# michaelklachko/NoisyNet

Measured on AMD Instinct MI355X. Metric: images/sec (whole node) + top-1, NoisyNet 4-bit CIFAR-10 I_max=1nA, 1/2/4/8 GPU, higher is better.
Workload: dtype bf16; 1 GPU; model=noisynet-4layer-cifar, global_batch=32768, image_size=32, augment=True, hip_graph=False, q_a=4, q_w=0, current_nA=1, act_max=5, optim=adamw, parallelism=dp1

## Files before the change

### __graft_entry__.py

```python
#!/usr/bin/env python3

import glob
import os
import shutil
import sys

REPO = os.path.dirname(os.path.abspath(__file__))
sys.path.insert(0, REPO)


def build():
    os.environ.setdefault("PYTORCH_ROCM_ARCH", "gfx950")

    sources = sorted(glob.glob(os.path.join(REPO, "csrc", "*.hip")))
    sources += sorted(glob.glob(os.path.join(REPO, "csrc", "*.cpp")))
    build_dir = os.path.join(REPO, "build")
    os.makedirs(build_dir, exist_ok=True)
    _build_manual(build_dir, sources)

    so_src = os.path.join(build_dir, "noisynet_hip.so")
    so_dst = os.path.join(REPO, "noisynet_amd", "ops", "noisynet_hip.so")
    if os.path.exists(so_src):
        shutil.copy2(so_src, so_dst)

    import noisynet_amd

    from noisynet_amd.ops import _ext
    mod = _ext.ext()
    for sym in ("conv_fwd_fused", "conv_wgrad_patch", "set_seed_buffer",
                "softmax_xent_bwd_t", "bn_stats_finalize", "dwconv_wgrad",
                "crop_resize_mirror_normalize", "conv_fused_route",
                "linear_fused_route", "xbar_fwd_conv", "xbar_fwd_linear",
                "xbar_diff_fwd_conv", "xbar_diff_fwd_linear",
                "xbar_serial_fwd_conv", "xbar_serial_fwd_linear"):
        if not hasattr(mod, sym):
            raise RuntimeError("build(): %s missing from %s -- stale build"
                               % (sym, so_dst))
    print("build(): extension built at", so_dst)


def _build_manual(build_dir, sources):
    import subprocess

    import torch
    from torch.utils import cpp_extension as ce

    torch_lib = os.path.join(os.path.dirname(torch.__file__), "lib")
    includes = ce.include_paths(device_type="cuda")
    inc_flags = ["-I" + p for p in includes]
# ... 104 lines not shown
```

### csrc/bindings.cpp

```cpp

#include <torch/extension.h>

torch::Tensor fake_quant_fwd(torch::Tensor x, int64_t num_bits, double min_value,
                             double max_value, double stochastic, int64_t seed);
torch::Tensor ste_mask(torch::Tensor grad, torch::Tensor x, double min_value,
                       double max_value);
torch::Tensor mult_uniform_noise(torch::Tensor x, double a, int64_t seed);
torch::Tensor relu_clip_fwd(torch::Tensor x, bool relu, double act_max);
torch::Tensor relu_clip_bwd(torch::Tensor g, torch::Tensor y, bool relu,
                            double act_max);
std::vector<torch::Tensor> dropout_fwd(torch::Tensor x, double p, int64_t seed);
void set_seed_buffer(torch::Tensor t);
void clear_seed_buffer();

void sgd_step(torch::Tensor p, torch::Tensor g, torch::Tensor buf, double lr,
              double momentum, double wd, bool nesterov, double cmin,
              double cmax);
void adamw_step(torch::Tensor p, torch::Tensor g, torch::Tensor m,
                torch::Tensor v, int64_t step, double lr, double beta1,
                double beta2, double eps, double wd, double cmin, double cmax);

std::vector<torch::Tensor> softmax_xent_fwd(torch::Tensor logits,
                                            torch::Tensor target);
torch::Tensor softmax_xent_bwd(torch::Tensor softmax, torch::Tensor target,
// ... 12 lines not shown
std::vector<torch::Tensor> bn_act_bwd(torch::Tensor g, torch::Tensor x,
                                      torch::Tensor y, torch::Tensor mean,
                                      torch::Tensor invstd, torch::Tensor gamma,
                                      bool training, bool relu,
                                      double act_max);
std::vector<torch::Tensor> bn_act_bwd_reduce(torch::Tensor g, torch::Tensor x,
                                             torch::Tensor y, torch::Tensor mean,
                                             torch::Tensor invstd, bool relu,
                                             double act_max);
torch::Tensor bn_act_bwd_apply(torch::Tensor g, torch::Tensor x,
                               torch::Tensor y, torch::Tensor mean,
                               torch::Tensor invstd, torch::Tensor gamma,
                               torch::Tensor sum_g, torch::Tensor sum_gx,
                               double count, bool training, bool relu,
                               double act_max);

std::vector<torch::Tensor> maxpool2x2_fwd(torch::Tensor x);
torch::Tensor maxpool2x2_bwd(torch::Tensor g, torch::Tensor code, int64_t H,
                             int64_t W);
std::vector<torch::Tensor> maxpool_fwd(torch::Tensor x, int64_t k,
                                       int64_t stride, int64_t pad);
torch::Tensor maxpool_bwd(torch::Tensor g, torch::Tensor code, int64_t H,
                          int64_t W, int64_t k, int64_t stride, int64_t pad);
torch::Tensor avgpool_fwd(torch::Tensor x, int64_t k, int64_t stride,
                          int64_t pad);
torch::Tensor avgpool_bwd(torch::Tensor g, int64_t H, int64_t W, int64_t k,
                          int64_t stride, int64_t pad);

torch::Tensor dwconv_fwd(torch::Tensor x, torch::Tensor w, torch::Tensor bias,
                         int64_t stride, int64_t pad);
// ... 13 lines not shown
                                           torch::Tensor meta,
                                           int64_t out_size,
                                           std::vector<double> mean,
                                           std::vector<double> std,
                                           int64_t out_dtype);

torch::Tensor kth_percentile(torch::Tensor x, double pctl);

torch::Tensor conv_fwd(torch::Tensor x, torch::Tensor w, int64_t stride,
                       int64_t pad);
std::vector<torch::Tensor> conv_fwd_fused(torch::Tensor x, torch::Tensor wq,
                                          torch::Tensor wraw, torch::Tensor bias,
                                          int64_t stride, int64_t pad,
                                          int64_t sigma_mode,
                                          torch::Tensor factor,
                                          int64_t seed, bool telem);
torch::Tensor conv_dgrad(torch::Tensor gy, torch::Tensor w, int64_t stride,
                         int64_t pad, int64_t H, int64_t W);
torch::Tensor conv_wgrad(torch::Tensor gy, torch::Tensor x, int64_t stride,
                         int64_t pad, int64_t R, int64_t S);
torch::Tensor im2col_materialize(torch::Tensor x, int64_t K, int64_t stride,
                                 int64_t pad, int64_t R, int64_t S);
torch::Tensor conv_wgrad_from_col(torch::Tensor gy, torch::Tensor col,
                                  int64_t C, int64_t R, int64_t S);
torch::Tensor conv_wgrad_im2col(torch::Tensor gy, torch::Tensor x,
                                int64_t stride, int64_t pad, int64_t R,
                                int64_t S);
torch::Tensor conv_wgrad_patch(torch::Tensor gy, torch::Tensor x,
                               int64_t stride, int64_t pad, int64_t R,
                               int64_t S,
                               c10::optional<torch::Tensor> x_padded);
// ... 80 lines not shown
  m.def("relu_clip_bwd", &relu_clip_bwd);
  m.def("dropout_fwd", &dropout_fwd);
  m.def("set_seed_buffer", &set_seed_buffer);
  m.def("clear_seed_buffer", &clear_seed_buffer);
  m.def("sgd_step", &sgd_step);
  m.def("adamw_step", &adamw_step);
  m.def("softmax_xent_fwd", &softmax_xent_fwd);
  m.def("softmax_xent_bwd", &softmax_xent_bwd);
  m.def("softmax_xent_bwd_t", &softmax_xent_bwd_t);
  m.def("bn_stats", &bn_stats);
  m.def("bn_stats_finalize", &bn_stats_finalize);
  m.def("bn_act_fwd", &bn_act_fwd);
  m.def("bn_act_bwd", &bn_act_bwd);
  m.def("bn_act_bwd_reduce", &bn_act_bwd_reduce);
  m.def("bn_act_bwd_apply", &bn_act_bwd_apply);
  m.def("maxpool2x2_fwd", &maxpool2x2_fwd);
  m.def("maxpool2x2_bwd", &maxpool2x2_bwd);
  m.def("dwconv_fwd", &dwconv_fwd);
  m.def("dwconv_dgrad", &dwconv_dgrad);
  m.def("dwconv_wgrad", &dwconv_wgrad);
  m.def("act_fwd", &act_fwd);
  m.def("act_bwd", &act_bwd);
  m.def("se_scale_fwd", &se_scale_fwd);
  m.def("se_scale_bwd", &se_scale_bwd);
  m.def("maxpool_fwd", &maxpool_fwd);
  m.def("maxpool_bwd", &maxpool_bwd);
  m.def("avgpool_fwd", &avgpool_fwd);
  m.def("avgpool_bwd", &avgpool_bwd);
  m.def("kth_percentile", &kth_percentile);
  m.def("crop_resize_mirror_normalize", &crop_resize_mirror_normalize);
  m.def("conv_fwd", &conv_fwd);
  m.def("conv_fwd_fused", &conv_fwd_fused);
  m.def("conv_dgrad", &conv_dgrad);
  m.def("conv_wgrad", &conv_wgrad);
  m.def("conv_wgrad_im2col", &conv_wgrad_im2col);
  m.def("conv_wgrad_patch", &conv_wgrad_patch, py::arg("gy"), py::arg("x"),
        py::arg("stride"), py::arg("pad"), py::arg("R"), py::arg("S"),
        py::arg("x_padded") = py::none());
  m.def("conv_wgrad_route", &conv_wgrad_route);
  m.def("conv_wgrad_from_col", &conv_wgrad_from_col);
  m.def("conv_pool_eligible", &conv_pool_eligible);
  m.def("conv_fused_route", &conv_fused_route);
  m.def("linear_fused_route", &linear_fused_route);
  m.def("conv_patch_tile", &conv_patch_tile);
  m.def("conv_pool_fwd_fused", &conv_pool_fwd_fused);
  m.def("conv_pool_wgrad", &conv_pool_wgrad);
  m.def("im2col_materialize", &im2col_materialize);
// ... 14 lines not shown
```

### csrc/bn_act.hip

```cpp

#include <torch/extension.h>
#include <ATen/ATen.h>
#include <c10/hip/HIPStream.h>
#include "common.h"

namespace {

constexpr int kBlock = 256;

template <typename T>
struct alignas(16) BnPack8 { T v[8]; };

template <typename T>
__global__ void bn_stats_kernel(const T* __restrict__ x,
                                float* __restrict__ partial_sum,
                                float* __restrict__ partial_sumsq,
                                int64_t rows, int C) {
  __shared__ float ls[kBlock], lsq[kBlock];
  int cbase = blockIdx.x * 64;
  int cw = C - cbase;
  if (cw > 64) cw = 64;
  int c_l = (cw == 64) ? (threadIdx.x & 63) : (threadIdx.x % cw);
  int rgrp = (cw == 64) ? (threadIdx.x >> 6) : (threadIdx.x / cw);
  int ngrp = kBlock / cw;
// ... 129 lines not shown
    outa[c] = sa;
    outb[c] = sb;
  }
}

template <typename T>
__global__ void bn_act_fwd_kernel(const T* __restrict__ x, T* __restrict__ y,
                                  const float* __restrict__ mean,
                                  const float* __restrict__ invstd,
                                  const float* __restrict__ gamma,
                                  const float* __restrict__ beta, int64_t n,
                                  int C, int do_relu, float act_max) {
  for (int64_t i = (int64_t)blockIdx.x * blockDim.x + threadIdx.x; i < n;
       i += (int64_t)gridDim.x * blockDim.x) {
    int c = (int)(i % C);
    float v = (to_f32(x[i]) - mean[c]) * invstd[c] * gamma[c] + beta[c];
    if (do_relu) v = fmaxf(v, 0.0f);
    if (act_max > 0.0f) v = fminf(v, act_max);
    y[i] = from_f32<T>(v);
  }
}

template <typename T>
__global__ void bn_act_fwd_vec_kernel(const T* __restrict__ x,
                                      T* __restrict__ y,
                                      const float* __restrict__ mean,
                                      const float* __restrict__ invstd,
                                      const float* __restrict__ gamma,
                                      const float* __restrict__ beta,
                                      int64_t n_vec, int Cv, int do_relu,
                                      float act_max) {
  using V = BnPack8<T>;
  for (int64_t i = (int64_t)blockIdx.x * blockDim.x + threadIdx.x; i < n_vec;
       i += (int64_t)gridDim.x * blockDim.x) {
    int c0 = (int)(i % Cv) * 8;
    V xv = ((const V*)x)[i];
    V o;
#pragma unroll
    for (int u = 0; u < 8; ++u) {
      int c = c0 + u;
      float v = (to_f32(xv.v[u]) - mean[c]) * invstd[c] * gamma[c] + beta[c];
      if (do_relu) v = fmaxf(v, 0.0f);
      if (act_max > 0.0f) v = fminf(v, act_max);
      o.v[u] = from_f32<T>(v);
    }
    ((V*)y)[i] = o;
  }
}

template <typename scalar_t> struct DevT { using type = scalar_t; };
template <> struct DevT<at::BFloat16> { using type = __hip_bfloat16; };
template <> struct DevT<at::Half> { using type = _Float16; };

__global__ void bn_finalize_kernel(const float* __restrict__ partial_sum,
                                   const float* __restrict__ partial_sumsq,
                                   float* __restrict__ mean,
                                   float* __restrict__ invstd,
                                   float* __restrict__ running_mean,
                                   float* __restrict__ running_var, int gy,
// ... 651 lines not shown
```

### csrc/common.h

```cpp
#pragma once

#include <hip/hip_runtime.h>
#include <hip/hip_bf16.h>
#include <hip/hip_fp16.h>
#include <cmath>
#include <cstdint>

#define WAVE 64
#define DEV_INLINE __device__ __forceinline__

template <typename T> DEV_INLINE float to_f32(T v);
template <> DEV_INLINE float to_f32<float>(float v) { return v; }
template <> DEV_INLINE float to_f32<__hip_bfloat16>(__hip_bfloat16 v) {
  return __bfloat162float(v);
}
template <> DEV_INLINE float to_f32<_Float16>(_Float16 v) { return (float)v; }

template <typename T> DEV_INLINE T from_f32(float v);
template <> DEV_INLINE float from_f32<float>(float v) { return v; }
template <> DEV_INLINE __hip_bfloat16 from_f32<__hip_bfloat16>(float v) {
  return __float2bfloat16(v);
}
template <> DEV_INLINE _Float16 from_f32<_Float16>(float v) {
  return (_Float16)v;
}

template <typename scalar_t>
inline float stored_act_max(double act_max) {
  return static_cast<float>(
      static_cast<scalar_t>(static_cast<float>(act_max)));
}

struct Philox4 {
  uint32_t x, y, z, w;
};

DEV_INLINE uint32_t mulhilo(uint32_t a, uint32_t b, uint32_t* hip) {
  uint64_t p = (uint64_t)a * (uint64_t)b;
  *hip = (uint32_t)(p >> 32);
  return (uint32_t)p;
}

DEV_INLINE Philox4 philox4x32(uint64_t seed, uint64_t counter) {
  uint32_t c0 = (uint32_t)counter, c1 = (uint32_t)(counter >> 32);
  uint32_t c2 = 0u, c3 = 0u;
// ... 106 lines not shown
```

### csrc/conv_mfma.hip

```cpp

#include <torch/extension.h>
#include <ATen/ATen.h>
#include <c10/hip/HIPStream.h>
#include <cstdlib>
#include <cstring>
#include <string>
#include "common.h"

namespace {

constexpr int kBlock = 256;
constexpr int BM = 64;
constexpr int BN = 64;
constexpr int BK = 32;

using bf16 = __hip_bfloat16;
using bf16x8 = __attribute__((ext_vector_type(8))) __bf16;
using f16x8 = __attribute__((ext_vector_type(8))) _Float16;
using f32x4 = __attribute__((ext_vector_type(4))) float;
using f32x8 = __attribute__((ext_vector_type(8))) float;


template <typename T> struct Mma;

// ... 2394 lines not shown
  } else {
    TORCH_CHECK(false, "conv_fwd_patch: layer-fitted tiles are 16-bit only");
  }
}

torch::Tensor pad_cols8(const torch::Tensor& in, int64_t K8);

bool conv_pad_share_enabled() {
  const char* e = getenv("NOISYNET_CONV_PAD_SHARE");
  return e == nullptr || std::string(e) != "0";
}

std::vector<torch::Tensor> conv_fwd_fused_patch_impl(
    torch::Tensor x, torch::Tensor wq, torch::Tensor wraw, torch::Tensor bias,
    int64_t stride, int64_t pad, int64_t sigma_mode, torch::Tensor factor,
    int64_t seed, bool telem, bool want_y) {
  check_sigma_mode(sigma_mode, want_y, "conv_fwd_fused (patch route)");
  check_cl(x, "conv_fwd_patch x");
  auto g = make_geom((int)x.size(0), (int)x.size(2), (int)x.size(3),
                     (int)x.size(1), (int)wraw.size(0), (int)wraw.size(2),
                     (int)wraw.size(3), (int)stride, (int)pad);
  PatchGeom p;
  p.C_pad = (g.C + 7) & ~7;
  p.Wp = g.W + 2 * g.pad;
  p.Kr = g.S * p.C_pad;
  p.Krs = (p.Kr + 31) & ~31;
  p.MI = g.OH * g.OW;
  auto out = torch::empty({g.N, g.K, g.OH, g.OW},
                          x.options().memory_format(at::MemoryFormat::ChannelsLast));
  bool has_bias = bias.numel() > 0;
  torch::Tensor bias_f;
  if (has_bias) bias_f = bias.to(torch::kFloat32).contiguous();
  auto tele = telem
      ? [&] {
          auto t = torch::zeros({3}, x.options().dtype(torch::kFloat32));
          t[2] = -std::numeric_limits<float>::infinity();
          return t;
        }()
      : torch::empty({0}, x.options().dtype(torch::kFloat32));
  auto factor_f = factor.to(torch::kFloat32).reshape({1}).contiguous();
  const PatchTileChoice tile = patch_tile(g, (int)x.element_size(),
                                          (int)sigma_mode, telem, want_y);
  torch::Tensor x_pad = torch::empty({0}, x.options());
  if (want_y && sigma_mode > 0 && x.element_size() == 2 && (g.C & 7) != 0 &&
      conv_pad_share_enabled()) {
    x_pad = pad_cols8(x.permute({0, 2, 3, 1})
                          .reshape({(int64_t)g.N * g.H * g.W, (int64_t)g.C})
                          .contiguous(), p.C_pad);
    x = x_pad;
    g.C = p.C_pad;
  }
  int k_pad = tile.kind == PatchTile::Generic ? (g.K + BN - 1) / BN * BN
                                              : tile.nrows;
  auto wq_pad = want_y ? pad_weight_full(wq, p.C_pad, k_pad, p.Krs)
                       : torch::Tensor();
  auto wraw_pad = (sigma_mode > 0)
                      ? pad_weight_full(wraw, p.C_pad, k_pad, p.Krs)
                      : torch::Tensor();
  size_t lds = 0;
  dim3 grid((g.K + BN - 1) / BN, g.N);
// ... 84 lines not shown
  } else {
    r = sigma_noise_linear_impl(col, wraw_flat, sigma_mode, factor, seed,
                                telem);
  }
  auto out = r[0].view({g.N, g.OH, g.OW, g.K}).permute({0, 3, 1, 2});
  return {out, r[1], col};
}

}

std::vector<torch::Tensor> conv_fwd_fused(torch::Tensor x, torch::Tensor wq,
                                          torch::Tensor wraw, torch::Tensor bias,
                                          int64_t stride, int64_t pad,
                                          int64_t sigma_mode,
                                          torch::Tensor factor,
                                          int64_t seed, bool telem) {
  auto g = make_geom((int)x.size(0), (int)x.size(2), (int)x.size(3),
                     (int)x.size(1), (int)wraw.size(0), (int)wraw.size(2),
                     (int)wraw.size(3), (int)stride, (int)pad);
  auto empty = torch::empty({0}, x.options());
  switch (conv_route(g, (int)x.element_size())) {
    case ConvRoute::Patch: {
      auto r = conv_fwd_fused_patch_impl(x, wq, wraw, bias, stride, pad,
                                         sigma_mode, factor, seed, telem,
                                         true);
      return r;
    }
    case ConvRoute::ColSmallK:
    case ConvRoute::ColGemm:
      return conv_fwd_fused_col_impl(x, wq, wraw, bias, stride, pad,
                                     sigma_mode, factor, seed, telem,
                                     true);
    case ConvRoute::Stream:
      break;
  }
  auto r = conv_fwd_fused_impl(x, wq, wraw, bias, stride, pad, sigma_mode,
                               factor, seed, telem, true);
  return {r[0], r[1], empty};
}

// ... 350 lines not shown
}

std::string conv_wgrad_route(int64_t C, int64_t H, int64_t W, int64_t K,
                             int64_t R, int64_t S, int64_t stride,
                             int64_t pad, int64_t elem_size) {
  if (ww_forced_legacy()) return "legacy";
  return ww_plan(1, C, H, W, K, R, S, stride, pad, elem_size, nullptr)
             ? "window" : "legacy";
}

torch::Tensor conv_wgrad_patch(torch::Tensor gy, torch::Tensor x,
                               int64_t stride, int64_t pad, int64_t R,
                               int64_t S,
                               c10::optional<torch::Tensor> x_padded) {
  check_cl(gy, "conv_wgrad_patch gy");
  check_cl(x, "conv_wgrad_patch x");
  TORCH_CHECK(x.element_size() == 2, "conv_wgrad_patch: 16-bit only");
  int64_t N = x.size(0), C = x.size(1), H = x.size(2), W = x.size(3);
  int64_t K = gy.size(1), OH = gy.size(2), OW = gy.size(3);
  int64_t M = N * OH * OW;
  int64_t Cp = (C + 7) & ~7;
  int64_t CRSp = R * S * Cp;

  auto x2 = x.permute({0, 2, 3, 1}).reshape({N * H * W, C});
  torch::Tensor xp;
  if (x_padded.has_value() && x_padded->numel() > 0) {
    TORCH_CHECK(x_padded->dim() == 2 && x_padded->size(0) == N * H * W &&
                    x_padded->size(1) == Cp && x_padded->is_contiguous() &&
                    x_padded->scalar_type() == x.scalar_type() &&
                    x_padded->device() == x.device(),
                "conv_wgrad_patch: x_padded must be [N*H*W, round8(C)]");
    xp = *x_padded;
  } else {
    xp = (Cp == C) ? x2.contiguous() : pad_cols8(x2.contiguous(), Cp);
  }
  auto gy2 = gy.permute({0, 2, 3, 1}).reshape({M, K});
  int64_t Kp = (K + 7) & ~7;
  torch::Tensor gyp = (Kp == K) ? gy2.contiguous()
                                : pad_cols8(gy2.contiguous(), Kp);

  int ctiles = (int)((CRSp + 127) / 128);
  int ktiles = (int)((Kp + 127) / 128);
  int64_t mtotal = (M + WG_BK - 1) / WG_BK;
  int64_t target_z = std::max<int64_t>(1, 2048 / std::max(1, ctiles * ktiles));
  int chunks = (int)((mtotal + target_z - 1) / target_z);
  int mslices = (int)((mtotal + chunks - 1) / chunks);
  dim3 grid(ctiles, ktiles, mslices);
  size_t lds = (size_t)256 * WG_LSTR;
// ... 1209 lines not shown
```

### noisynet_amd/models/noisynet.py

```python

import torch
from torch import nn

from .. import ops
from ..hardware_model import NoisyConv2d, NoisyLinear, add_noise_calculate_power
from ..quant import QuantMeasure


class Net(nn.Module):
    def __init__(self, args=None):
        super().__init__()
        self.args = args
        self.create_dir = True

        if args.train_act_max:
            self.act_max1 = nn.Parameter(torch.Tensor([0]), requires_grad=True)
            self.act_max2 = nn.Parameter(torch.Tensor([0]), requires_grad=True)
            self.act_max3 = nn.Parameter(torch.Tensor([0]), requires_grad=True)
        if args.train_w_max:
            self.w_max1 = nn.Parameter(torch.Tensor([0]), requires_grad=True)
            self.w_min1 = nn.Parameter(torch.Tensor([0]), requires_grad=True)

        self.pool = nn.MaxPool2d(2, 2)
        self.relu = nn.ReLU()
# ... 110 lines not shown
                                         -(-q_a // 4)))
        flags = self._introspective_flags()
        if flags:
            raise ValueError(
                '--xbar_rows %d cannot be combined with --%s: that flag runs '
                'the introspective forward, which models one unbounded '
                'crossbar per layer' % (self.xbar_rows, flags[0]))

    def _conv1_pool_fused(self, x, i):
        a = self.args
        return (a.current1 > 0 and i >= 20 and not x.requires_grad
                and a.L3 == 0 and a.L4 == 0
                and getattr(a, 'L3_new', 0) == 0
                and ops.conv_pool_eligible(x, self.conv1.weight))

    def _noisy_layer_fused(self, x, layer, current, merged_dac, i, layer_num,
                           is_conv, pool=False):
        a = self.args
        w_raw = layer.weight
        wq, bias = layer.effective_weight()
        want_telemetry = i < 20
        with torch.no_grad():
            if merged_dac:
                w_max = w_raw.detach().abs().max()
                factor = 0.1 * w_max / current
                sigma_mode = 'abs'
                power_denom = (x.detach().max() * w_max if want_telemetry
                               else w_max)
            else:
                input_max = x.detach().max()
                factor = 0.1 * input_max / current
                sigma_mode = 'abs2'
                power_denom = input_max
        telem = ops.NoiseTelemetry() if want_telemetry else None
        if is_conv:
            conv = ops.fused_noisy_conv2d_pool if pool \
                else ops.fused_noisy_conv2d
            out = conv(
                x, wq, w_raw.detach(), bias, 1, 0, sigma_mode, factor,
                current=current, power_denom=power_denom,
                want_telemetry=want_telemetry, telemetry_out=telem)
        else:
            out = ops.fused_noisy_linear(
                x, wq, w_raw.detach(), bias, sigma_mode, factor,
                current=current, power_denom=power_denom,
                want_telemetry=want_telemetry, telemetry_out=telem)
        if want_telemetry and telem.power is not None:
            self.power[layer_num].append(float(telem.power))
            self.nsr[layer_num].append(float(telem.nsr))
            self.input_sparsity[layer_num].append(float(telem.input_sparsity))
        return out

    def _xbar_serial_args(self, layer_num):
        if self.xbar_dac_bits <= 0:
            return {}
        k = layer_num + 1
# ... 83 lines not shown
                                 args.merged_dac, i, 0, True)
            self.conv1_ = x
            x = ops.maxpool2x2(x)
        elif self._conv1_pool_fused(x, i):
            x = self._noisy_layer_fused(x, self.conv1, args.current1,
                                        args.merged_dac, i, 0, True, pool=True)
            self.conv1_ = None
        else:
            if args.current1 > 0:
                x = self._noisy_layer_fused(x, self.conv1, args.current1,
                                            args.merged_dac, i, 0, True)
            else:
                x = self.conv1(x)
            self.conv1_ = x
            x = ops.maxpool2x2(x)
        if args.batchnorm:
            x = self._bn_act(x, self.bn1, args.act_max1)
        else:
            x = ops.relu_clip(x, args.act_max1)
        if args.dropout_conv > 0:
            x = ops.dropout(x, args.dropout_conv, self.training)
        if args.q_a2 > 0:
            x = self.quantize2(x)

        if xbar:
            x = self._xbar_layer(x, self.conv2, args.current2, False, i, 1,
                                 True)
        elif args.current2 > 0:
            x = self._noisy_layer_fused(x, self.conv2, args.current2,
                                        False, i, 1, True)
        else:
            x = self.conv2(x)
        self.conv2_ = x
        x = ops.maxpool2x2(x)
        if args.batchnorm:
            x = self._bn_act(x, self.bn2, args.act_max2)
        else:
            x = ops.relu_clip(x, args.act_max2)
        if args.dropout > 0:
            x = ops.dropout(x, args.dropout, self.training)
# ... 220 lines not shown
```

### noisynet_amd/ops/__init__.py

```python
from . import reference
from ._ext import ext, has_ext, use_native
from .functional import (
    adamw_step,
    add_weight_noise,
    bn_act,
    conv2d,
    crop_resize_mirror_normalize,
    cross_entropy,
    depthwise_conv2d,
    dropout,
    fake_quant,
    hard_sigmoid,
    hard_swish,
    conv_pool_eligible,
    fused_noisy_conv2d,
    fused_noisy_conv2d_pool,
    fused_noisy_linear,
    avgpool_nhwc,
    kth_percentile,
    linear,
    maxpool2x2,
    maxpool_nhwc,
    per_sample_conv2d,
    se_scale,
# ... 14 lines not shown
```

### noisynet_amd/ops/functional.py

```python

import os as _os

import torch
import torch.nn.functional as F

from . import reference as ref
from ._ext import ext, use_native


def _next_seed(device):
    return int(torch.randint(0, 2 ** 62, (1,), device="cpu").item())




class FakeQuant(torch.autograd.Function):

    @staticmethod
    def forward(ctx, x, num_bits, min_value, max_value, stochastic):
        ctx.min_value = float(min_value)
        ctx.max_value = float(max_value)
        ctx.save_for_backward(x)
        if use_native(x):
            return ext().fake_quant_fwd(
# ... 78 lines not shown
                                x_shape[2], x_shape[3])
    return torch.nn.grad.conv2d_input(x_shape, w, g, stride, padding)


def _is_padded_input(shared, x):
    C = x.shape[1]
    return (shared is not None and shared.dim() == 2 and C % 8 != 0
            and shared.shape[0] == x.shape[0] * x.shape[2] * x.shape[3]
            and shared.shape[1] == (C + 7) // 8 * 8)


def _conv_wgrad_raw(g, x, stride, padding, w_shape, col=None):
    if use_native(g, x):
        R, S = w_shape[2], w_shape[3]
        if _is_padded_input(col, x):
            return ext().conv_wgrad_patch(_nhwc(g), _nhwc(x), stride,
                                          padding, R, S, col)
        if col is not None and R * S > 1 \
                and not _os.environ.get("NOISYNET_WGRAD_NO_COL"):
            return ext().conv_wgrad_from_col(_nhwc(g), col, x.shape[1], R, S)
        if R * S > 1 and x.element_size() == 2:
            return ext().conv_wgrad_patch(_nhwc(g), _nhwc(x), stride,
                                          padding, R, S)
        if R * S == 1 and stride == 1 and padding == 0:
            gn, xn = _nhwc(g), _nhwc(x)
            K = gn.shape[1]
            C_in = xn.shape[1]
            m = gn.shape[0] * gn.shape[2] * gn.shape[3]
            g2 = gn.permute(0, 2, 3, 1).reshape(m, K)
            x2 = xn.permute(0, 2, 3, 1).reshape(m, C_in)
            dw = ext().linear_wgrad(g2.contiguous(), x2.contiguous())
# ... 83 lines not shown

class NoiseTelemetry:

    __slots__ = ("power", "nsr", "input_sparsity")

    def __init__(self, power=None, nsr=None, input_sparsity=None):
        self.power = power
        self.nsr = nsr
        self.input_sparsity = input_sparsity


class _FusedNoisyConv(torch.autograd.Function):

    @staticmethod
    def forward(ctx, x, wq, w_raw, bias, stride, padding, sigma_mode, factor,
                want_telemetry, telemetry_out, current, power_denom):
        ctx.stride, ctx.padding = stride, padding
        ctx.has_bias = bias is not None
        col = None
        if use_native(x, wq):
            y, tele, col = ext().conv_fwd_fused(
                _nhwc(x), _nhwc(wq), _nhwc(w_raw),
                bias if bias is not None else torch.empty(0, device=x.device, dtype=x.dtype),
                stride, padding, 1 if sigma_mode == "abs" else 2,
                _factor_tensor(factor, x.device), _next_seed(x.device),
                bool(want_telemetry))
            if want_telemetry:
                sum_sigma_abs = tele[0] / x.shape[0]
                sum_abs_noise = tele[1] / y.numel()
                max_y = tele[2]
        else:
            y = F.conv2d(x, wq, bias, stride, padding)
            with torch.no_grad():
                sig = ref.sigma_conv2d(x.detach(), w_raw, sigma_mode, stride, padding)
                noise = ref.vmm_noise(sig, factor)
                if want_telemetry:
                    if sigma_mode == "abs":
                        sig_abs = sig
                    else:
                        sig_abs = ref.sigma_conv2d(x.detach(), w_raw, "abs", stride, padding)
                    sum_sigma_abs = sig_abs.sum(dim=(1, 2, 3)).mean()
# ... 10 lines not shown
        else:
            ctx.save_for_backward(x, wq)
        return y

    @staticmethod
    def backward(ctx, g):
        x, wq = ctx.saved_tensors[0], ctx.saved_tensors[1]
        col = ctx.saved_tensors[2] if len(ctx.saved_tensors) > 2 else None
        gx = gw = gb = None
        if ctx.needs_input_grad[0]:
            gx = ConvDgrad.apply(g, wq, ctx.stride, ctx.padding, x.shape)
        if ctx.needs_input_grad[1]:
            gw = ConvWgrad.apply(g, x, ctx.stride, ctx.padding, wq.shape, col)
        if ctx.has_bias and ctx.needs_input_grad[3]:
            gb = g.sum(dim=(0, 2, 3))
        return (gx, gw, None, gb) + (None,) * 8


def fused_noisy_conv2d(x, wq, w_raw, bias, stride, padding, sigma_mode,
                       factor, current=0.0, power_denom=1.0,
                       want_telemetry=False, telemetry_out=None):
    return _FusedNoisyConv.apply(x, wq, w_raw, bias, stride, padding,
                                 sigma_mode, factor, want_telemetry,
                                 telemetry_out, current, power_denom)




def conv_pool_eligible(x, w, stride=1, padding=0):
    if _os.environ.get("NOISYNET_NO_CONV1_POOL"):
        return False
    if not use_native(x, w) or stride != 1 or padding != 0:
        return False
    if x.dtype != w.dtype or x.dim() != 4:
        return False
    return bool(ext().conv_pool_eligible(
        x.shape[1], x.shape[2], x.shape[3], w.shape[0], w.shape[2],
        w.shape[3], x.element_size()))

# ... 561 lines not shown
                g - g_beta_r.view(shape) / n - xhat * g_gamma_r.view(shape) / n)
        else:
            gx = g * (wf.view(shape) * invstd.view(shape))
        return (gx.to(x.dtype), g_gamma.to(weight.dtype),
                g_beta.to(weight.dtype)) + (None,) * 8


def bn_act(x, weight, bias, running_mean, running_var, training, momentum,
           eps, relu=True, act_max=0.0, sync=False):
    return BnAct.apply(x, weight, bias, running_mean, running_var, training,
                       momentum, eps, relu, act_max, sync)




class MaxPool2x2(torch.autograd.Function):
    @staticmethod
    def forward(ctx, x):
        if use_native(x):
            y, idx = ext().maxpool2x2_fwd(_nhwc(x))
        else:
            y, idx = F.max_pool2d(x, 2, 2, return_indices=True)
        ctx.save_for_backward(idx)
        ctx.x_shape = x.shape
        return y

    @staticmethod
    def backward(ctx, g):
        (idx,) = ctx.saved_tensors
        if use_native(g):
# ... 499 lines not shown
```

### noisynet_amd/quant.py

```python

import torch
from torch import nn

from . import ops


class UniformQuantize(torch.autograd.Function):

    @staticmethod
    def forward(ctx, input, num_bits=8, min_value=None, max_value=None,
                stochastic=0.5, inplace=False, debug=False):
        ctx.min_value = min_value
        ctx.max_value = max_value
        ctx.save_for_backward(input)
        with torch.no_grad():
            return ops.reference.fake_quant_forward(
                input, num_bits, min_value, max_value, stochastic
            ) if not input.is_cuda else ops.ext().fake_quant_fwd(
                input, int(num_bits), float(min_value), float(max_value),
                float(stochastic),
                int(torch.randint(0, 2 ** 62, (1,)).item()))

    @staticmethod
    def backward(ctx, grad_output):
# ... 24 lines not shown
        self.max_value = max_value
        self.min_value = min_value
        self.scale = scale
        self.calculate_running = calculate_running
        self.running_list = []
        self.pctl = pctl
        self._range_cache = None
        self.last_range = None
        if pctl < 1:
            raise ValueError('pctl is {} please check'.format(pctl))

    def _load_from_state_dict(self, *args, **kwargs):
        self._range_cache = None
        return super()._load_from_state_dict(*args, **kwargs)

    def forward(self, input):
        with torch.no_grad():
            min_value = self.min_value
            max_value = self.max_value
            if self.calculate_running:
                if self.min_value < 0:
                    pos = input[input > 0]
                    neg = input[input < 0].abs()
                    pctl_pos = ops.kth_percentile(pos, self.pctl)
                    pctl_neg = ops.kth_percentile(neg, self.pctl)
                    self.running_min = -pctl_neg.reshape(1)
                    self.running_max = pctl_pos.reshape([])
                    self.calculate_running = False
                    min_value = float(self.running_min.item())
                    max_value = float(self.running_max.item())
                else:
                    if 224 in list(input.shape):
                        if self.num_bits == 4:
                            pctl_val = torch.tensor(0.92)
                        else:
# ... 2 lines not shown
                        pctl_val = ops.kth_percentile(input, self.pctl)
                    max_value = input.max().item()
                    self.running_list.append(pctl_val)
            elif self._range_cache is not None:
                min_value, max_value = self._range_cache
            else:
                cacheable = True
                if self.min_value < 0 and float(self.running_min.min()) < 0:
                    min_value = float(self.running_min.item())
                    max_value = float(self.running_max.item())
                elif self.max_value > 0:
                    max_value = self.max_value
                elif float(self.running_max) > 0:
                    max_value = float(self.running_max)
                else:
                    max_value = input.max().item()
                    cacheable = False
                if cacheable:
                    self._range_cache = (min_value, max_value)

            stoch = self.stochastic if self.training else 0
            self.last_range = (float(min_value), float(max_value))

        return ops.fake_quant(input, self.num_bits, min_value, max_value, stoch)


def finish_calibration(model, device=None):
    with torch.no_grad():
        for m in model.modules():
            if isinstance(m, QuantMeasure):
                m._range_cache = None
                if m.calculate_running and m.running_list:
                    m.calculate_running = False
                    vals = torch.stack([torch.as_tensor(v, dtype=torch.float32)
                                        for v in m.running_list])
                    m.running_max = vals.mean().to(
                        device if device is not None else m.running_max.device)

# ... 7 lines not shown
```

Measured before the change: 1.102 million images/sec.

## Fuse batchnorm, ReLU-clip and activation quantization into one kernel emitting padded conv input

Adds a bn_act_quant_fwd kernel that applies batchnorm, ReLU and clip, then fake-quantizes in a single pass. It also writes the quantized output directly in the channel-padded layout the next patch conv expects, and records the max via atomics. The conv forward accepts this pre-padded tensor, so it skips its own pad_cols8 copy, and wgrad uses it too. This removes separate elementwise passes, an extra full read/write of the activation, and the pad copy. In exchange the kernel is more complex, keeps both act and quantized outputs, and adds LDS staging for the padded path.

```diff
diff --git a/__graft_entry__.py b/__graft_entry__.py
--- a/__graft_entry__.py
+++ b/__graft_entry__.py
@@ -32,7 +32,8 @@
                 "crop_resize_mirror_normalize", "conv_fused_route",
                 "linear_fused_route", "xbar_fwd_conv", "xbar_fwd_linear",
                 "xbar_diff_fwd_conv", "xbar_diff_fwd_linear",
-                "xbar_serial_fwd_conv", "xbar_serial_fwd_linear"):
+                "xbar_serial_fwd_conv", "xbar_serial_fwd_linear",
+                "bn_act_quant_fwd"):
         if not hasattr(mod, sym):
             raise RuntimeError("build(): %s missing from %s -- stale build"
                                % (sym, so_dst))
diff --git a/csrc/bindings.cpp b/csrc/bindings.cpp
--- a/csrc/bindings.cpp
+++ b/csrc/bindings.cpp
@@ -50,6 +50,11 @@
                                torch::Tensor sum_g, torch::Tensor sum_gx,
                                double count, bool training, bool relu,
                                double act_max);
+std::vector<torch::Tensor> bn_act_quant_fwd(
+    torch::Tensor x, torch::Tensor mean, torch::Tensor invstd,
+    torch::Tensor gamma, torch::Tensor beta, bool relu, double act_max,
+    int64_t num_bits, double min_value, double max_value, double stochastic,
+    int64_t seed, int64_t C_pad);
 
 std::vector<torch::Tensor> maxpool2x2_fwd(torch::Tensor x);
 torch::Tensor maxpool2x2_bwd(torch::Tensor g, torch::Tensor code, int64_t H,
@@ -93,7 +98,8 @@
                                           int64_t stride, int64_t pad,
                                           int64_t sigma_mode,
                                           torch::Tensor factor,
-                                          int64_t seed, bool telem);
+                                          int64_t seed, bool telem,
+                                          c10::optional<torch::Tensor> x_padded);
 torch::Tensor conv_dgrad(torch::Tensor gy, torch::Tensor w, int64_t stride,
                          int64_t pad, int64_t H, int64_t W);
 torch::Tensor conv_wgrad(torch::Tensor gy, torch::Tensor x, int64_t stride,
@@ -204,6 +210,7 @@
   m.def("bn_act_bwd", &bn_act_bwd);
   m.def("bn_act_bwd_reduce", &bn_act_bwd_reduce);
   m.def("bn_act_bwd_apply", &bn_act_bwd_apply);
+  m.def("bn_act_quant_fwd", &bn_act_quant_fwd);
   m.def("maxpool2x2_fwd", &maxpool2x2_fwd);
   m.def("maxpool2x2_bwd", &maxpool2x2_bwd);
   m.def("dwconv_fwd", &dwconv_fwd);
@@ -220,7 +227,10 @@
   m.def("kth_percentile", &kth_percentile);
   m.def("crop_resize_mirror_normalize", &crop_resize_mirror_normalize);
   m.def("conv_fwd", &conv_fwd);
-  m.def("conv_fwd_fused", &conv_fwd_fused);
+  m.def("conv_fwd_fused", &conv_fwd_fused, py::arg("x"), py::arg("wq"),
+        py::arg("wraw"), py::arg("bias"), py::arg("stride"), py::arg("pad"),
+        py::arg("sigma_mode"), py::arg("factor"), py::arg("seed"),
+        py::arg("telem"), py::arg("x_padded") = py::none());
   m.def("conv_dgrad", &conv_dgrad);
   m.def("conv_wgrad", &conv_wgrad);
   m.def("conv_wgrad_im2col", &conv_wgrad_im2col);
diff --git a/csrc/bn_act.hip b/csrc/bn_act.hip
--- a/csrc/bn_act.hip
+++ b/csrc/bn_act.hip
@@ -167,10 +167,8 @@
   for (int64_t i = (int64_t)blockIdx.x * blockDim.x + threadIdx.x; i < n;
        i += (int64_t)gridDim.x * blockDim.x) {
     int c = (int)(i % C);
-    float v = (to_f32(x[i]) - mean[c]) * invstd[c] * gamma[c] + beta[c];
-    if (do_relu) v = fmaxf(v, 0.0f);
-    if (act_max > 0.0f) v = fminf(v, act_max);
-    y[i] = from_f32<T>(v);
+    y[i] = bn_act_value<T>(to_f32(x[i]), mean[c], invstd[c], gamma[c],
+                           beta[c], do_relu, act_max);
   }
 }
 
@@ -192,10 +190,8 @@
 #pragma unroll
     for (int u = 0; u < 8; ++u) {
       int c = c0 + u;
-      float v = (to_f32(xv.v[u]) - mean[c]) * invstd[c] * gamma[c] + beta[c];
-      if (do_relu) v = fmaxf(v, 0.0f);
-      if (act_max > 0.0f) v = fminf(v, act_max);
-      o.v[u] = from_f32<T>(v);
+      o.v[u] = bn_act_value<T>(to_f32(xv.v[u]), mean[c], invstd[c], gamma[c],
+                               beta[c], do_relu, act_max);
     }
     ((V*)y)[i] = o;
   }
diff --git a/csrc/bn_act_quant.hip b/csrc/bn_act_quant.hip
--- /dev/null
+++ b/csrc/bn_act_quant.hip
@@ -0,0 +1,240 @@
+
+#include <torch/extension.h>
+#include <ATen/ATen.h>
+#include <c10/hip/HIPStream.h>
+#include "common.h"
+
+namespace {
+
+constexpr int kBlock = 256;
+constexpr int kFwdGridCap = 2048;
+
+template <typename T>
+struct alignas(16) Pack8 { T v[8]; };
+
+template <typename scalar_t> struct DevT { using type = scalar_t; };
+template <> struct DevT<at::BFloat16> { using type = __hip_bfloat16; };
+template <> struct DevT<at::Half> { using type = _Float16; };
+
+DEV_INLINE int pidx(int c) { return c + (c >> 3); }
+inline int pstride(int C) { return C + (C >> 3) + 1; }
+
+template <typename T, bool STOCH>
+DEV_INLINE T quant_value(T a, float u, float min_value, float inv_scale,
+                         float scale, float qmax) {
+#pragma clang fp contract(off)
+  float q = (to_f32(a) - min_value) * inv_scale;
+  if (STOCH) q = q + u;
+  q = fminf(fmaxf(q, 0.0f), qmax);
+  q = nearbyintf(q);
+  return from_f32<T>(__fmaf_rn(q, scale, min_value));
+}
+
+DEV_INLINE float quant_offset(uint32_t r, float stoch) {
+#pragma clang fp contract(off)
+  return __fmaf_rn(2.0f, u01(r), -1.0f) * stoch;
+}
+
+template <typename T, bool STOCH, bool PAD>
+__global__ void bn_act_quant_fwd_kernel(
+    const T* __restrict__ x, T* __restrict__ act, T* __restrict__ out,
+    int* __restrict__ max_bits,
+    const float* __restrict__ mean, const float* __restrict__ invstd,
+    const float* __restrict__ gamma, const float* __restrict__ beta,
+    int64_t rows, int C, int C_pad, int slab_rows, int ps, int do_relu,
+    float act_max, float min_value, float inv_scale, float scale, float qmax,
+    float stoch, uint64_t seed, const int64_t* __restrict__ seed_base) {
+  extern __shared__ __align__(16) char smem[];
+  __shared__ float wmax[kBlock / WAVE];
+  float* p_mean = (float*)smem;
+  float* p_is = p_mean + ps;
+  float* p_ga = p_is + ps;
+  float* p_be = p_ga + ps;
+  T* slab = (T*)(smem + (((size_t)4 * ps * sizeof(float) + 15) & ~(size_t)15));
+  for (int c = threadIdx.x; c < C; c += kBlock) {
+    p_mean[pidx(c)] = mean[c];
+    p_is[pidx(c)] = invstd[c];
+    p_ga[pidx(c)] = gamma[c];
+    p_be[pidx(c)] = beta[c];
+  }
+  __syncthreads();
+  seed = graph_seed(seed_base, seed);
+  const int nchunks = C_pad >> 3;
+  const int cstep = (kBlock * 8) % C;
+  float vmax = 0.0f;
+  for (int64_t r0 = (int64_t)blockIdx.x * slab_rows; r0 < rows;
+       r0 += (int64_t)gridDim.x * slab_rows) {
+    const int64_t e0 = r0 * C;
+    const int64_t r1 = r0 + slab_rows < rows ? r0 + slab_rows : rows;
+    const int64_t e1 = r1 * C;
+    int c = (threadIdx.x * 8) % C;
+    for (int64_t e = e0 + (int64_t)threadIdx.x * 8; e < e1;
+         e += kBlock * 8) {
+      const bool full = e + 8 <= e1;
+      Pack8<T> xv;
+      if (full) {
+        xv = *(const Pack8<T>*)(x + e);
+      } else {
+#pragma unroll
+        for (int j = 0; j < 8; ++j)
+          xv.v[j] = (e + j < e1) ? x[e + j] : from_f32<T>(0.0f);
+      }
+      float u[8] = {};
+      if (STOCH) {
+        Philox4 ph = philox4x32(seed, (uint64_t)(e >> 2));
+        u[0] = quant_offset(ph.x, stoch);
+        u[1] = quant_offset(ph.y, stoch);
+        u[2] = quant_offset(ph.z, stoch);
+        u[3] = quant_offset(ph.w, stoch);
+        if (e + 4 < e1) {
+          ph = philox4x32(seed, (uint64_t)(e >> 2) + 1);
+          u[4] = quant_offset(ph.x, stoch);
+          u[5] = quant_offset(ph.y, stoch);
+          u[6] = quant_offset(ph.z, stoch);
+          u[7] = quant_offset(ph.w, stoch);
+        }
+      }
+      Pack8<T> o, av;
+      int cc = c;
+#pragma unroll
+      for (int j = 0; j < 8; ++j) {
+        const int pi = pidx(cc);
+        T a = bn_act_value<T>(to_f32(xv.v[j]), p_mean[pi], p_is[pi], p_ga[pi],
+                              p_be[pi], do_relu, act_max);
+        av.v[j] = a;
+        o.v[j] = quant_value<T, STOCH>(a, u[j], min_value, inv_scale, scale,
+                                       qmax);
+        if (full || e + j < e1) vmax = fmaxf(vmax, to_f32(o.v[j]));
+        if (++cc == C) cc = 0;
+      }
+      T* dst = PAD ? slab + (e - e0) : out + e;
+      if (full) {
+        *(Pack8<T>*)dst = o;
+        *(Pack8<T>*)(act + e) = av;
+      } else {
+#pragma unroll
+        for (int j = 0; j < 8; ++j)
+          if (e + j < e1) {
+            dst[j] = o.v[j];
+            act[e + j] = av.v[j];
+          }
+      }
+      c += cstep;
+      if (c >= C) c -= C;
+    }
+    if (PAD) {
+      __syncthreads();
+      const int total = (int)(r1 - r0) * nchunks;
+      for (int t = threadIdx.x; t < total; t += kBlock) {
+        const int lr = t / nchunks;
+        const int base = (t - lr * nchunks) * 8;
+        Pack8<T> o;
+#pragma unroll
+        for (int j = 0; j < 8; ++j)
+          o.v[j] = (base + j < C) ? slab[lr * C + base + j]
+                                  : from_f32<T>(0.0f);
+        *(Pack8<T>*)(out + (r0 + lr) * (int64_t)C_pad + base) = o;
+      }
+      __syncthreads();
+    }
+  }
+  vmax = wave_max(vmax);
+  if ((threadIdx.x & (WAVE - 1)) == 0) wmax[threadIdx.x / WAVE] = vmax;
+  __syncthreads();
+  if (threadIdx.x == 0) {
+    float m = wmax[0];
+    for (int w = 1; w < kBlock / WAVE; ++w) m = fmaxf(m, wmax[w]);
+    atomicMax(max_bits, __float_as_int(m));
+  }
+}
+
+struct Shape {
+  int C;
+  int64_t rows;
+};
+
+Shape check_inputs(const char* fn, const torch::Tensor& x,
+                   std::initializer_list<torch::Tensor> per_c) {
+  TORCH_CHECK(x.is_cuda(), fn, ": expected a GPU tensor");
+  TORCH_CHECK(x.scalar_type() == torch::kBFloat16 ||
+                  x.scalar_type() == torch::kHalf,
+              fn, ": 16-bit dtypes only");
+  TORCH_CHECK(x.dim() == 4 || x.dim() == 2, fn, ": expected a 4-D or 2-D x");
+  Shape s;
+  if (x.dim() == 4) {
+    TORCH_CHECK(x.is_contiguous(at::MemoryFormat::ChannelsLast), fn,
+                ": expected channels_last x");
+    s.rows = x.size(0) * x.size(2) * x.size(3);
+  } else {
+    TORCH_CHECK(x.is_contiguous(), fn, ": expected contiguous x");
+    s.rows = x.size(0);
+  }
+  s.C = (int)x.size(1);
+  TORCH_CHECK(s.C >= 1 && s.rows >= 1, fn, ": empty input");
+
+  TORCH_CHECK(((uintptr_t)x.data_ptr() & 15) == 0, fn,
+              ": x must be 16-byte aligned");
+  for (const auto& t : per_c)
+    TORCH_CHECK(t.is_cuda() && t.scalar_type() == torch::kFloat32 &&
+                    t.is_contiguous() && t.numel() == s.C,
+                fn, ": per-channel tensors must be contiguous f32 [C] on the GPU");
+  return s;
+}
+
+}
+
+std::vector<torch::Tensor> bn_act_quant_fwd(
+    torch::Tensor x, torch::Tensor mean, torch::Tensor invstd,
+    torch::Tensor gamma, torch::Tensor beta, bool relu, double act_max,
+    int64_t num_bits, double min_value, double max_value, double stochastic,
+    int64_t seed, int64_t C_pad) {
+  const char* fn = "bn_act_quant_fwd";
+  Shape s = check_inputs(fn, x, {mean, invstd, gamma, beta});
+  TORCH_CHECK(relu && min_value == 0.0, fn,
+              ": needs relu and min_value == 0");
+  TORCH_CHECK(C_pad == s.C || (C_pad > s.C && (C_pad & 7) == 0), fn,
+              ": C_pad must be C or a multiple of 8 above it");
+  const bool pad = C_pad != s.C;
+  const int C = s.C;
+  const int ps = pstride(C);
+  const size_t par_bytes = ((size_t)4 * ps * sizeof(float) + 15) & ~(size_t)15;
+  int slab_rows = 64;
+  while (pad && slab_rows > 8 &&
+         par_bytes + (size_t)slab_rows * C * 2 > 48 * 1024)
+    slab_rows >>= 1;
+  const size_t lds = par_bytes + (pad ? (size_t)slab_rows * C * 2 : 0);
+  TORCH_CHECK(lds <= 64 * 1024, fn, ": C = ", C, " is too wide");
+  auto act = torch::empty_like(x);
+  auto out = torch::empty({s.rows, C_pad}, x.options());
+  auto maxv = torch::zeros({1}, x.options().dtype(torch::kFloat32));
+  float qmax = ::powf(2.0f, (float)num_bits) - 1.0f;
+  float scale = std::max(((float)max_value - (float)min_value) / qmax, 1e-6f);
+  int64_t nslabs = (s.rows + slab_rows - 1) / slab_rows;
+  int blocks = (int)std::min<int64_t>(nslabs, kFwdGridCap);
+  auto stream = c10::hip::getCurrentHIPStream();
+  NN_DISPATCH(x.scalar_type(), "bn_act_quant_fwd", [&] {
+    using T = typename DevT<scalar_t>::type;
+    if constexpr (sizeof(T) == 2) {
+      auto launch = [&](auto kfn, float st) {
+        hipLaunchKernelGGL(kfn, dim3(blocks), dim3(kBlock), lds, stream,
+                           (const T*)x.data_ptr(), (T*)act.data_ptr(),
+                           (T*)out.data_ptr(),
+                           (int*)maxv.data_ptr<float>(),
+                           mean.data_ptr<float>(), invstd.data_ptr<float>(),
+                           gamma.data_ptr<float>(), beta.data_ptr<float>(),
+                           s.rows, C, (int)C_pad, slab_rows, ps, 1,
+                           (float)act_max, (float)min_value, 1.0f / scale,
+                           scale, qmax, st, (uint64_t)seed, g_seed_base);
+      };
+      if (stochastic > 0) {
+        if (pad) launch(&bn_act_quant_fwd_kernel<T, true, true>, (float)stochastic);
+        else launch(&bn_act_quant_fwd_kernel<T, true, false>, (float)stochastic);
+      } else {
+        if (pad) launch(&bn_act_quant_fwd_kernel<T, false, true>, 0.0f);
+        else launch(&bn_act_quant_fwd_kernel<T, false, false>, 0.0f);
+      }
+    }
+  });
+  HIP_CHECK_LAST();
+  return {act, out, maxv};
+}
diff --git a/csrc/common.h b/csrc/common.h
--- a/csrc/common.h
+++ b/csrc/common.h
@@ -29,6 +29,16 @@
 inline float stored_act_max(double act_max) {
   return static_cast<float>(
       static_cast<scalar_t>(static_cast<float>(act_max)));
+}
+
+template <typename T>
+DEV_INLINE T bn_act_value(float xv, float mean, float invstd, float gamma,
+                          float beta, int do_relu, float act_max) {
+#pragma clang fp contract(off)
+  float v = __fmaf_rn((xv - mean) * invstd, gamma, beta);
+  if (do_relu) v = fmaxf(v, 0.0f);
+  if (act_max > 0.0f) v = fminf(v, act_max);
+  return from_f32<T>(v);
 }
 
 struct Philox4 {
diff --git a/csrc/conv_mfma.hip b/csrc/conv_mfma.hip
--- a/csrc/conv_mfma.hip
+++ b/csrc/conv_mfma.hip
@@ -2432,9 +2432,11 @@
 std::vector<torch::Tensor> conv_fwd_fused_patch_impl(
     torch::Tensor x, torch::Tensor wq, torch::Tensor wraw, torch::Tensor bias,
     int64_t stride, int64_t pad, int64_t sigma_mode, torch::Tensor factor,
-    int64_t seed, bool telem, bool want_y) {
+    int64_t seed, bool telem, bool want_y,
+    const c10::optional<torch::Tensor>& x_prepadded = c10::nullopt) {
   check_sigma_mode(sigma_mode, want_y, "conv_fwd_fused (patch route)");
-  check_cl(x, "conv_fwd_patch x");
+  const bool prepadded = x_prepadded.has_value() && x_prepadded->numel() > 0;
+  if (!prepadded) check_cl(x, "conv_fwd_patch x");
   auto g = make_geom((int)x.size(0), (int)x.size(2), (int)x.size(3),
                      (int)x.size(1), (int)wraw.size(0), (int)wraw.size(2),
                      (int)wraw.size(3), (int)stride, (int)pad);
@@ -2460,8 +2462,23 @@
   const PatchTileChoice tile = patch_tile(g, (int)x.element_size(),
                                           (int)sigma_mode, telem, want_y);
   torch::Tensor x_pad = torch::empty({0}, x.options());
-  if (want_y && sigma_mode > 0 && x.element_size() == 2 && (g.C & 7) != 0 &&
-      conv_pad_share_enabled()) {
+  const bool pad_route = want_y && sigma_mode > 0 && x.element_size() == 2 &&
+                         (g.C & 7) != 0 && conv_pad_share_enabled();
+  if (prepadded) {
+    TORCH_CHECK(pad_route,
+                "conv_fwd_fused: a pre-padded input is taken by the noisy "
+                "16-bit patch route with C % 8 != 0 only");
+    TORCH_CHECK(x_prepadded->dim() == 2 &&
+                    x_prepadded->size(0) == (int64_t)g.N * g.H * g.W &&
+                    x_prepadded->size(1) == p.C_pad &&
+                    x_prepadded->is_contiguous() &&
+                    x_prepadded->scalar_type() == x.scalar_type() &&
+                    x_prepadded->device() == x.device(),
+                "conv_fwd_fused: x_padded must be [N*H*W, round8(C)]");
+    x_pad = *x_prepadded;
+    x = x_pad;
+    g.C = p.C_pad;
+  } else if (pad_route) {
     x_pad = pad_cols8(x.permute({0, 2, 3, 1})
                           .reshape({(int64_t)g.N * g.H * g.W, (int64_t)g.C})
                           .contiguous(), p.C_pad);
@@ -2576,16 +2593,22 @@
                                           int64_t stride, int64_t pad,
                                           int64_t sigma_mode,
                                           torch::Tensor factor,
-                                          int64_t seed, bool telem) {
+                                          int64_t seed, bool telem,
+                                          c10::optional<torch::Tensor> x_padded) {
+  TORCH_CHECK(x.dim() == 4, "conv_fwd_fused: expected a 4-D x");
   auto g = make_geom((int)x.size(0), (int)x.size(2), (int)x.size(3),
                      (int)x.size(1), (int)wraw.size(0), (int)wraw.size(2),
                      (int)wraw.size(3), (int)stride, (int)pad);
   auto empty = torch::empty({0}, x.options());
-  switch (conv_route(g, (int)x.element_size())) {
+  const bool prepadded = x_padded.has_value() && x_padded->numel() > 0;
+  const ConvRoute route = conv_route(g, (int)x.element_size());
+  TORCH_CHECK(!prepadded || route == ConvRoute::Patch,
+              "conv_fwd_fused: a pre-padded input needs the patch route");
+  switch (route) {
     case ConvRoute::Patch: {
       auto r = conv_fwd_fused_patch_impl(x, wq, wraw, bias, stride, pad,
                                          sigma_mode, factor, seed, telem,
-                                         true);
+                                         true, x_padded);
       return r;
     }
     case ConvRoute::ColSmallK:
@@ -2966,7 +2989,12 @@
                                int64_t S,
                                c10::optional<torch::Tensor> x_padded) {
   check_cl(gy, "conv_wgrad_patch gy");
-  check_cl(x, "conv_wgrad_patch x");
+  const bool have_xp = x_padded.has_value() && x_padded->numel() > 0;
+  if (have_xp) {
+    TORCH_CHECK(x.dim() == 4, "conv_wgrad_patch x: expected a 4-D tensor");
+  } else {
+    check_cl(x, "conv_wgrad_patch x");
+  }
   TORCH_CHECK(x.element_size() == 2, "conv_wgrad_patch: 16-bit only");
   int64_t N = x.size(0), C = x.size(1), H = x.size(2), W = x.size(3);
   int64_t K = gy.size(1), OH = gy.size(2), OW = gy.size(3);
@@ -2974,9 +3002,8 @@
   int64_t Cp = (C + 7) & ~7;
   int64_t CRSp = R * S * Cp;
 
-  auto x2 = x.permute({0, 2, 3, 1}).reshape({N * H * W, C});
   torch::Tensor xp;
-  if (x_padded.has_value() && x_padded->numel() > 0) {
+  if (have_xp) {
     TORCH_CHECK(x_padded->dim() == 2 && x_padded->size(0) == N * H * W &&
                     x_padded->size(1) == Cp && x_padded->is_contiguous() &&
                     x_padded->scalar_type() == x.scalar_type() &&
@@ -2984,6 +3011,7 @@
                 "conv_wgrad_patch: x_padded must be [N*H*W, round8(C)]");
     xp = *x_padded;
   } else {
+    auto x2 = x.permute({0, 2, 3, 1}).reshape({N * H * W, C});
     xp = (Cp == C) ? x2.contiguous() : pad_cols8(x2.contiguous(), Cp);
   }
   auto gy2 = gy.permute({0, 2, 3, 1}).reshape({M, K});
diff --git a/noisynet_amd/models/noisynet.py b/noisynet_amd/models/noisynet.py
--- a/noisynet_amd/models/noisynet.py
+++ b/noisynet_amd/models/noisynet.py
@@ -148,8 +148,24 @@
                 and getattr(a, 'L3_new', 0) == 0
                 and ops.conv_pool_eligible(x, self.conv1.weight))
 
+    def _bn_quant_range(self, x, i):
+        import os
+        a = self.args
+        if not (self.training and a.batchnorm and i >= 20
+                and self.xbar_rows == 0 and a.q_a2 > 0 and a.current2 > 0
+                and a.dropout_conv == 0
+                and not getattr(a, 'sync_bn', False)
+                and not self.quantize2.calculate_running
+                and not os.environ.get('NOISYNET_NO_BN_QUANT_FUSE')
+                and ops.bn_act_quant_native(x, self.bn1.running_mean, 0.0)):
+            return None
+        rng = self.quantize2.quant_range()
+        if rng is None or rng[0] != 0:
+            return None
+        return rng
+
     def _noisy_layer_fused(self, x, layer, current, merged_dac, i, layer_num,
-                           is_conv, pool=False):
+                           is_conv, pool=False, x_pad=None, input_max=None):
         a = self.args
         w_raw = layer.weight
         wq, bias = layer.effective_weight()
@@ -162,7 +178,8 @@
                 power_denom = (x.detach().max() * w_max if want_telemetry
                                else w_max)
             else:
-                input_max = x.detach().max()
+                if input_max is None:
+                    input_max = x.detach().max()
                 factor = 0.1 * input_max / current
                 sigma_mode = 'abs2'
                 power_denom = input_max
@@ -170,10 +187,11 @@
         if is_conv:
             conv = ops.fused_noisy_conv2d_pool if pool \
                 else ops.fused_noisy_conv2d
+            extra = {} if x_pad is None else {'x_pad': x_pad}
             out = conv(
                 x, wq, w_raw.detach(), bias, 1, 0, sigma_mode, factor,
                 current=current, power_denom=power_denom,
-                want_telemetry=want_telemetry, telemetry_out=telem)
+                want_telemetry=want_telemetry, telemetry_out=telem, **extra)
         else:
             out = ops.fused_noisy_linear(
                 x, wq, w_raw.detach(), bias, sigma_mode, factor,
@@ -287,16 +305,29 @@
                 x = self.conv1(x)
             self.conv1_ = x
             x = ops.maxpool2x2(x)
-        if args.batchnorm:
-            x = self._bn_act(x, self.bn1, args.act_max1)
-        else:
-            x = ops.relu_clip(x, args.act_max1)
-        if args.dropout_conv > 0:
-            x = ops.dropout(x, args.dropout_conv, self.training)
-        if args.q_a2 > 0:
-            x = self.quantize2(x)
-
-        if xbar:
+        q2 = self._bn_quant_range(x, i)
+        if q2 is not None:
+            bn = self.bn1
+            x, x_pad, x_max = ops.bn_act_quant(
+                x, bn.weight, bn.bias, bn.running_mean, bn.running_var,
+                bn.momentum, bn.eps, args.act_max1, args.q_a2, q2[0], q2[1],
+                q2[2], c_pad=ops.conv_input_pad_width(x, self.conv2.weight))
+            x = self._noisy_layer_fused(x, self.conv2, args.current2, False,
+                                        i, 1, True, x_pad=x_pad,
+                                        input_max=x_max)
+        else:
+            if args.batchnorm:
+                x = self._bn_act(x, self.bn1, args.act_max1)
+            else:
+                x = ops.relu_clip(x, args.act_max1)
+            if args.dropout_conv > 0:
+                x = ops.dropout(x, args.dropout_conv, self.training)
+            if args.q_a2 > 0:
+                x = self.quantize2(x)
+
+        if q2 is not None:
+            pass
+        elif xbar:
             x = self._xbar_layer(x, self.conv2, args.current2, False, i, 1,
                                  True)
         elif args.current2 > 0:
diff --git a/noisynet_amd/ops/__init__.py b/noisynet_amd/ops/__init__.py
--- a/noisynet_amd/ops/__init__.py
+++ b/noisynet_amd/ops/__init__.py
@@ -4,6 +4,9 @@
     adamw_step,
     add_weight_noise,
     bn_act,
+    bn_act_quant,
+    bn_act_quant_native,
+    conv_input_pad_width,
     conv2d,
     crop_resize_mirror_normalize,
     cross_entropy,
diff --git a/noisynet_amd/ops/functional.py b/noisynet_amd/ops/functional.py
--- a/noisynet_amd/ops/functional.py
+++ b/noisynet_amd/ops/functional.py
@@ -116,7 +116,7 @@
     if use_native(g, x):
         R, S = w_shape[2], w_shape[3]
         if _is_padded_input(col, x):
-            return ext().conv_wgrad_patch(_nhwc(g), _nhwc(x), stride,
+            return ext().conv_wgrad_patch(_nhwc(g), x, stride,
                                           padding, R, S, col)
         if col is not None and R * S > 1 \
                 and not _os.environ.get("NOISYNET_WGRAD_NO_COL"):
@@ -230,17 +230,20 @@
 
     @staticmethod
     def forward(ctx, x, wq, w_raw, bias, stride, padding, sigma_mode, factor,
-                want_telemetry, telemetry_out, current, power_denom):
+                want_telemetry, telemetry_out, current, power_denom,
+                x_pad=None):
         ctx.stride, ctx.padding = stride, padding
         ctx.has_bias = bias is not None
         col = None
+        if x_pad is not None and not use_native(x, wq):
+            raise ValueError("fused_noisy_conv2d: x_pad is a GPU-route argument")
         if use_native(x, wq):
             y, tele, col = ext().conv_fwd_fused(
-                _nhwc(x), _nhwc(wq), _nhwc(w_raw),
+                x if x_pad is not None else _nhwc(x), _nhwc(wq), _nhwc(w_raw),
                 bias if bias is not None else torch.empty(0, device=x.device, dtype=x.dtype),
                 stride, padding, 1 if sigma_mode == "abs" else 2,
                 _factor_tensor(factor, x.device), _next_seed(x.device),
-                bool(want_telemetry))
+                bool(want_telemetry), x_pad)
             if want_telemetry:
                 sum_sigma_abs = tele[0] / x.shape[0]
                 sum_abs_noise = tele[1] / y.numel()
@@ -281,15 +284,15 @@
             gw = ConvWgrad.apply(g, x, ctx.stride, ctx.padding, wq.shape, col)
         if ctx.has_bias and ctx.needs_input_grad[3]:
             gb = g.sum(dim=(0, 2, 3))
-        return (gx, gw, None, gb) + (None,) * 8
+        return (gx, gw, None, gb) + (None,) * 9
 
 
 def fused_noisy_conv2d(x, wq, w_raw, bias, stride, padding, sigma_mode,
                        factor, current=0.0, power_denom=1.0,
-                       want_telemetry=False, telemetry_out=None):
+                       want_telemetry=False, telemetry_out=None, x_pad=None):
     return _FusedNoisyConv.apply(x, wq, w_raw, bias, stride, padding,
                                  sigma_mode, factor, want_telemetry,
-                                 telemetry_out, current, power_denom)
+                                 telemetry_out, current, power_denom, x_pad)
 
 
 
@@ -881,6 +884,84 @@
 
 
 
+def conv_input_pad_width(x, w, padding=0):
+    C = x.shape[1]
+    if (C % 8 == 0 or not use_native(x, w) or x.element_size() != 2
+            or _os.environ.get("NOISYNET_CONV_PAD_SHARE") == "0"):
+        return C
+    route = ext().conv_fused_route(C, x.shape[2], x.shape[3], w.shape[0],
+                                   w.shape[2], w.shape[3], 1, padding,
+                                   x.element_size())
+    return (C + 7) // 8 * 8 if route == "patch" else C
+
+
+def bn_act_quant_native(x, running_mean, min_value):
+    return (use_native(x) and x.dtype in (torch.bfloat16, torch.float16)
+            and x.dim() in (2, 4) and x.numel() > 0 and x.numel() % 4 == 0
+            and (running_mean is None or running_mean.dtype == torch.float32)
+            and float(min_value) == 0.0)
+
+
+class BnActQuant(torch.autograd.Function):
+
+    @staticmethod
+    def forward(ctx, x, weight, bias, running_mean, running_var, momentum,
+                eps, act_max, num_bits, min_value, max_value, stochastic,
+                c_pad):
+        xc = _nhwc(x) if x.dim() == 4 else x.contiguous()
+        empty = torch.empty(0, device=x.device, dtype=torch.float32)
+        mean, invstd = ext().bn_stats_finalize(
+            xc,
+            running_mean if running_mean is not None else empty,
+            running_var if running_var is not None else empty,
+            float(momentum), float(eps))
+        act, xq_pad, xmax = ext().bn_act_quant_fwd(
+            xc, mean, invstd, weight.float().contiguous(),
+            bias.float().contiguous(), True, float(act_max), int(num_bits),
+            float(min_value), float(max_value), float(stochastic),
+            _next_seed(x.device), int(c_pad))
+        C = x.shape[1]
+        if x.dim() == 4:
+            N, _, H, W = x.shape
+            xq = xq_pad.view(N, H, W, c_pad)[..., :C].permute(0, 3, 1, 2)
+        else:
+            xq = xq_pad[:, :C]
+        xmax = xmax.to(x.dtype).reshape(())
+        ctx.save_for_backward(xc, weight, mean, invstd, act)
+        ctx.act_max = float(act_max)
+        ctx.q_range = (float(min_value), float(max_value))
+        ctx.mark_non_differentiable(xq_pad, xmax)
+        return xq, xq_pad, xmax
+
+    @staticmethod
+    def backward(ctx, g, _g_pad, _g_max):
+        x, weight, mean, invstd, act = ctx.saved_tensors
+        gq = ext().ste_mask(g, act, ctx.q_range[0], ctx.q_range[1])
+        gx, g_gamma, g_beta = ext().bn_act_bwd(
+            gq, x, act, mean, invstd, weight.float().contiguous(), True, True,
+            ctx.act_max)
+        return (gx, g_gamma.to(weight.dtype),
+                g_beta.to(weight.dtype)) + (None,) * 10
+
+
+def bn_act_quant(x, weight, bias, running_mean, running_var, momentum, eps,
+                 act_max, num_bits, min_value, max_value, stochastic=0.0,
+                 c_pad=None):
+    C = x.shape[1]
+    if bn_act_quant_native(x, running_mean, min_value):
+        c_pad = C if c_pad is None else int(c_pad)
+        xq, xq_pad, xmax = BnActQuant.apply(
+            x, weight, bias, running_mean, running_var, momentum, eps,
+            act_max, num_bits, min_value, max_value, stochastic, c_pad)
+        return xq, (xq_pad if c_pad != C else None), xmax
+    y = bn_act(x, weight, bias, running_mean, running_var, True, momentum,
+               eps, relu=True, act_max=act_max)
+    xq = fake_quant(y, num_bits, min_value, max_value, stochastic)
+    return xq, None, xq.detach().max()
+
+
+
+
 class MaxPool2x2(torch.autograd.Function):
     @staticmethod
     def forward(ctx, x):
diff --git a/noisynet_amd/quant.py b/noisynet_amd/quant.py
--- a/noisynet_amd/quant.py
+++ b/noisynet_amd/quant.py
@@ -62,11 +62,13 @@
         self._range_cache = None
         return super()._load_from_state_dict(*args, **kwargs)
 
-    def forward(self, input):
+    def quant_range(self, input=None):
         with torch.no_grad():
             min_value = self.min_value
             max_value = self.max_value
             if self.calculate_running:
+                if input is None:
+                    return None
                 if self.min_value < 0:
                     pos = input[input > 0]
                     neg = input[input < 0].abs()
@@ -99,6 +101,8 @@
                 elif float(self.running_max) > 0:
                     max_value = float(self.running_max)
                 else:
+                    if input is None:
+                        return None
                     max_value = input.max().item()
                     cacheable = False
                 if cacheable:
@@ -106,7 +110,10 @@
 
             stoch = self.stochastic if self.training else 0
             self.last_range = (float(min_value), float(max_value))
+        return min_value, max_value, stoch
 
+    def forward(self, input):
+        min_value, max_value, stoch = self.quant_range(input)
         return ops.fake_quant(input, self.num_bits, min_value, max_value, stoch)
 
 
```

Measured after the change: 1.169 million images/sec, median of 6. 1.06x the previous value.
